# choyingw/SynergyNet

Hardware: AMD Instinct MI355X
Metric: faces/sec (120x120, 68-lmk + 53215-vert) (higher is better)
Workload: dtype f32 (fp16x2 split operands, fp32 accumulate)

## Files before the change

### synergynet_amd/csrc/fused_block_rm.hip

```cpp
#include "syn_internal.h"

#include <cstdlib>

namespace syn {

typedef float f32x4 __attribute__((ext_vector_type(4)));
typedef float f32x16 __attribute__((ext_vector_type(16)));
typedef unsigned u32x4 __attribute__((ext_vector_type(4)));
typedef _Float16 f16x8 __attribute__((ext_vector_type(8)));
typedef _Float16 f16x2 __attribute__((ext_vector_type(2)));

namespace {
constexpr int cdivr(int a, int b) { return (a + b - 1) / b; }

__device__ __forceinline__ void split2r(float x0, float x1, unsigned &a, unsigned &b) {
    a = __builtin_bit_cast(unsigned, __builtin_amdgcn_cvt_pkrtz(x0, x1));
    float r0, r1;
    asm("v_fma_mix_f32 %0, %1, -1.0, %2 op_sel_hi:[1,0,0]" : "=v"(r0) : "v"(a), "v"(x0));
    asm("v_fma_mix_f32 %0, %1, -1.0, %2 op_sel:[1,0,0] op_sel_hi:[1,0,0]" : "=v"(r1) : "v"(a), "v"(x1));
    b = __builtin_bit_cast(unsigned, __builtin_amdgcn_cvt_pkrtz(r0, r1));
}
__device__ __forceinline__ f32x16 mfma32r(u32x4 a, u32x4 b, f32x16 c) {
    return __builtin_amdgcn_mfma_f32_32x32x16_f16(__builtin_bit_cast(f16x8, a), __builtin_bit_cast(f16x8, b), c, 0, 0, 0);
}
__device__ __forceinline__ f32x16 mac3r(const u32x4 (&a)[2], const u32x4 (&b)[2], f32x16 c) {
// ... 14 lines not shown
struct RmCfg {
    static constexpr bool SVC2 = SVC2_;
    static constexpr int NSVW = SVC2_ ? 2 * U_ : U_;
    static constexpr int CIN = CIN_, HID = HID_, COUT = COUT_, H = H_, S = S_, NF = NF_, WPE = WPE_, U = U_;
    static constexpr bool RES = RES_;
    static constexpr bool LEAN = LEAN_;
    static constexpr int WREG = WREG_;
    static constexpr int KS = cdivr(CIN, 16);
    static constexpr int NG = cdivr(HID, 32);
    static constexpr int HIDP = NG * 32;
    static constexpr int NQ = COUT / 8;
    static constexpr int NB = S == 1 ? 1 : 2;
    static constexpr int HO = S == 2 ? H / 2 : H;
    static constexpr int NBD = NBD_, HB = HO / NBD;
    static constexpr int BSTEPS = S == 1 ? cdivr(HB + 2, 3) * 3 : 2 * (HB + 1);
    static_assert(HO % NBD == 0 && (NBD == 1 || !LEAN_), "bands: equal heights; not implemented for the one-slot (LEAN) sums");
    static_assert(!SVC2_ || NBD_ == 1, "two service waves per unit: implemented for the whole-face march");
    static constexpr int NW = NG, NCW = U * NG, NT = (NCW + NSVW) * 64;
    static constexpr int FR = NB * KS;
    static constexpr int XP_DW = FR * 2 * 256, PART_DW = NW * NQ * 256;
    static constexpr int PSLOTS = LEAN ? 1 : 2;
    static constexpr int UNIT_DW = 2 * XP_DW + PSLOTS * PART_DW;
    static constexpr int APL_DW = LEAN ? NG * 2 * 2 * 256 : 0;
    static constexpr int LDS_DW = U * UNIT_DW + 11 * HIDP + 32 + APL_DW;
    static_assert(COUT % 8 == 0 && COUT <= 32, "project tile");
    static_assert(S == 1 || H % 2 == 0, "stride-2 blocks have even input sizes");
    static_assert(S == 1 ? (NF == 1 ? H + 2 <= 32 : 2 * H + 2 <= 32) : (NF == 1 ? H / 2 + 1 <= 32 : H / 2 + 1 <= 16), "one image row per 32-lane block");
    static_assert(!RES || (S == 1 && CIN == COUT), "residual only on stride-1 same-width blocks");
    static_assert(!LEAN || S == 1, "LEAN is implemented for the stride-1 march");
    static_assert(WREG == 0 || (S == 1 && WREG <= 4), "the register-held filter is implemented for the stride-1 march");
    static_assert(S == 2 || H % 3 == 0, "row ring unrolled by 3");
    static_assert(NT <= 1024 && LDS_DW * 4 <= 160 * 1024, "workgroup size / LDS budget");
};

#define SYNR_LAP(i) do { if (PROF) { tn = __builtin_amdgcn_s_memtime(); pt_[i] += tn - tk; tk = tn; } } while (0)
#define SYNR_BARRIER() do { if (PROF) { const unsigned long long tb_ = __builtin_amdgcn_s_memtime(); busy_ += tb_ - tw_; __syncthreads(); tw_ = __builtin_amdgcn_s_memtime(); } else __syncthreads(); } while (0)

template <class C, bool PROF>
__device__ __forceinline__ void rm_block(unsigned *smem, const float *__restrict__ X, const unsigned *__restrict__ Ae3 ,
                           const unsigned *__restrict__ Ap3 , const float *__restrict__ e_shift,
                           const float *__restrict__ Wd , const float *__restrict__ d_shift,
                           const float *__restrict__ p_shift, float *__restrict__ Y, int B, int ub_begin, int ub_end, int ub_step ,
                           const float *__restrict__ scl_e , const float *__restrict__ scl_p,
                           unsigned long long *prof) {
    unsigned long long pt_[7] = {0, 0, 0, 0, 0, 0, 0}, tk = PROF ? __builtin_amdgcn_s_memtime() : 0ull, tn = 0, nsteps = 0;
    const unsigned long long t_begin = tk;
    unsigned long long busy_ = 0, tw_ = tk;
    constexpr int H = C::H, HO = C::HO, NW = C::NW, NT = C::NT;
    const int tid = threadIdx.x, lane = tid & 63;
    const int wave_wg = __builtin_amdgcn_readfirstlane(tid >> 6);
    const bool service = wave_wg >= C::NCW;
    const int uw = service ? (wave_wg - C::NCW) % C::U : wave_wg / NW;
    const bool svc_in = !C::SVC2 || wave_wg - C::NCW < C::U, svc_out = !C::SVC2 || wave_wg - C::NCW >= C::U;
    const int wave = service ? 0 : wave_wg % NW;
    unsigned *Xp = smem + uw * C::UNIT_DW;
    float *Part = reinterpret_cast<float *>(Xp + 2 * C::XP_DW);
    float *Filt = reinterpret_cast<float *>(smem + C::U * C::UNIT_DW);
    float *Esh = Filt + 10 * C::HIDP, *Psh = Esh + C::HIDP;
    unsigned *ApL = reinterpret_cast<unsigned *>(Psh + 32);
    constexpr int DSH = 9 * C::HIDP;
    const int j = lane & 31, h = lane >> 5;
    const int cb = wave * 32 + 4 * h;
    const int nq_live = (C::HID % 32 == 16 && wave == NW - 1) ? 2 : 4;

    int ia, icol[C::NB], oa, ocol;
    if (C::S == 1 && C::NF == 2) {
        ia = j > C::H; icol[0] = (j == 0 || j == C::H + 1) ? -1 : j - 1 - (C::H + 1) * ia; oa = ia; ocol = icol[0];
    } else if (C::S == 1) { ia = 0; icol[0] = j - 1; oa = 0; ocol = j - 1; }
    else if (C::NF == 1) { ia = 0; icol[0] = 2 * j - 1; icol[C::NB - 1] = 2 * j; oa = 0; ocol = j; }
    else { ia = j >> 4; icol[0] = 2 * (j & 15) - 1; icol[C::NB - 1] = 2 * (j & 15); oa = j >> 4; ocol = j & 15; }
    u32x4 ae[C::KS][2], ap[2][2];
    unsigned early_sink = 0;
    if (!service) {
#pragma unroll
        for (int s = 0; s < C::KS; ++s)
#pragma unroll
            for (int p = 0; p < 2; ++p) ae[s][p] = *(const u32x4 *)(Ae3 + ((size_t)(wave * C::KS + s) * 2 + p) * 256 + lane * 4);
        if (!C::LEAN)
#pragma unroll
            for (int s = 0; s < 2; ++s)
#pragma unroll
                for (int p = 0; p < 2; ++p) ap[s][p] = *(const u32x4 *)(Ap3 + ((size_t)(wave * 2 + s) * 2 + p) * 256 + lane * 4);
    } else if (svc_in && ub_begin < ub_end) {
        const int unit = ub_begin + uw, fu = C::NBD > 1 ? unit / C::NBD : unit, r0 = C::NBD > 1 ? (unit - fu * C::NBD) * C::HB : 0;
        const int f_in = fu * C::NF + ia, y0 = C::NBD > 1 ? (C::S == 1 ? r0 - 1 : 2 * (r0 - 1)) : 0;
#pragma unroll
        for (int b = 0; b < C::NB; ++b)
#pragma unroll
            for (int yy = 0; yy < 2; ++yy) {
                const int y = y0 + yy;
                if ((unsigned)icol[b] < (unsigned)H && f_in < B && (unsigned)y < (unsigned)H) {
                    const float *src = X + ((size_t)(f_in * H + y) * H + icol[b]) * C::CIN + 8 * h;
                    asm volatile("global_load_dword %0, %1, off" : "+v"(early_sink) : "v"(src) : "memory");
                }
            }
    }
    const float Se = scl_e[0], c6e = scl_e[1] * (1.0f / 6.0f), inv_sp = scl_p[1] * 6.0f;
    for (int i = tid; i < 9 * C::HIDP; i += NT) { const int c = i % C::HIDP; Filt[i] = c < C::HID ? Wd[(i / C::HIDP) * C::HID + c] : 0.f; }
    for (int i = tid; i < C::HIDP; i += NT) { Filt[DSH + i] = i < C::HID ? d_shift[i] * (1.0f / 6.0f) : 0.f; Esh[i] = i < C::HID ? e_shift[i] * Se : 0.f; }
    if (tid < 32) Psh[tid] = tid < C::COUT ? p_shift[tid] : 0.f;
    if (C::LEAN)
        for (int i = tid; i < C::APL_DW / 4; i += NT) *(u32x4 *)&ApL[4 * i] = *(const u32x4 *)&Ap3[4 * i];

    __syncthreads();
    l2_touch_done(early_sink);

    if (service) {
        __builtin_amdgcn_s_setprio(3);
        for (int ub = ub_begin; ub < ub_end; ub += ub_step) {
            const int unit = ub + uw;
            const int fu = C::NBD > 1 ? unit / C::NBD : unit, r0 = C::NBD > 1 ? (unit - fu * C::NBD) * C::HB : 0;
            const int f_in = fu * C::NF + ia, f_out = fu * C::NF + oa;
            const bool out_ok = (unsigned)ocol < (unsigned)HO && f_out < B;
            f32x4 xr[C::FR][2];
            auto load_row = [&](int y) {
#pragma unroll
                for (int fr = 0; fr < C::FR; ++fr) {
                    const int b = fr / C::KS, sk = fr % C::KS, c0 = 16 * sk + 8 * h;
                    xr[fr][0] = (f32x4){0.f, 0.f, 0.f, 0.f}; xr[fr][1] = xr[fr][0];
                    if (c0 + 8 <= C::CIN && (unsigned)icol[b] < (unsigned)H && f_in < B && (C::NBD == 1 || (unsigned)y < (unsigned)H)) {
                        const float *src = X + ((size_t)(f_in * H + y) * H + icol[b]) * C::CIN + c0;
                        xr[fr][0] = *(const f32x4 *)src; xr[fr][1] = *(const f32x4 *)(src + 4);
                    }
                }
            };
            auto store_row = [&](int slot) {
#pragma unroll
                for (int fr = 0; fr < C::FR; ++fr) {
                    u32x4 pc[2];
#pragma unroll
                    for (int t = 0; t < 2; ++t) {
                        unsigned a0, b0, a1, b1;
                        split2r(xr[fr][t][0], xr[fr][t][1], a0, b0);
                        split2r(xr[fr][t][2], xr[fr][t][3], a1, b1);
                        pc[0][2 * t] = a0; pc[0][2 * t + 1] = a1; pc[1][2 * t] = b0; pc[1][2 * t + 1] = b1;
                    }
                    unsigned *dst = Xp + (size_t)slot * C::XP_DW + fr * 512 + lane * 4;
#pragma unroll
                    for (int p = 0; p < 2; ++p) *(u32x4 *)(dst + p * 256) = pc[p];
                }
            };
            f32x4 res[C::RES ? C::NQ : 1];
            auto load_res = [&](int yo) {
                if (C::RES) {
#pragma unroll
                    for (int q = 0; q < C::NQ; ++q) {
                        res[q] = (f32x4){0.f, 0.f, 0.f, 0.f};
                        if (out_ok && yo >= 0 && yo < HO) res[q] = *(const f32x4 *)(X + ((size_t)(f_out * H + yo) * H + ocol) * C::CIN + 8 * q + 4 * h);
// ... 14 lines not shown
            };
            if (C::NBD > 1) {
                constexpr int NS = C::BSTEPS, HB = C::HB;
                const int gy0 = C::S == 1 ? r0 - 1 : 2 * (r0 - 1);
                load_row(gy0);
                store_row(0);
                load_row(gy0 + 1);
                SYNR_BARRIER();
                for (int k = 0; k < NS; ++k) {
                    if (C::S == 1) {
                        if (k >= 3 && k < HB + 3) reduce_row(r0 + k - 3, (k - 1) & 1);
                        if (k >= 2) load_res(r0 + k - 2);
                    } else {
                        if (!(k & 1) && k >= 4) reduce_row(r0 + (k >> 1) - 2, ((k >> 1) - 1) & 1);
                    }
                    if (k + 1 < NS) store_row((k + 1) & 1);
                    if (k + 2 < NS) load_row(gy0 + k + 2);
                    SYNR_BARRIER();
                }
                if (C::S == 2) reduce_row(r0 + HB - 1, HB & 1);
                else if (NS == HB + 2) reduce_row(r0 + HB - 1, (NS - 1) & 1);
                continue;
            }
            if (svc_in) { load_row(0); store_row(0); load_row(1); }
            SYNR_BARRIER();
            if (C::S == 1) {
                if (svc_out) load_res(0);
                constexpr int PM = C::PSLOTS - 1;
                for (int y = 0; y < H; ++y) {
                    if (svc_out && y >= 2) reduce_row(y - 2, y & PM);
                    if (C::LEAN) SYNR_BARRIER();
                    if (svc_out) load_res(y - 1);
                    if (svc_in && y + 1 < H) store_row((y + 1) & 1);
                    if (svc_in && y + 2 < H) load_row(y + 2);
                    SYNR_BARRIER();
                }
                if (svc_out) reduce_row(H - 2, (H - 2) & PM);
                if (C::LEAN) SYNR_BARRIER();
                if (svc_out) load_res(H - 1);
                SYNR_BARRIER();
                if (svc_out) reduce_row(H - 1, (H - 1) & PM);
            } else {
                for (int y = 0; y < H; ++y) {
                    if (svc_out && !(y & 1) && y >= 2) reduce_row((y >> 1) - 1, ((y >> 1) - 1) & 1);
                    if (svc_in && y + 1 < H) store_row((y + 1) & 1);
                    if (svc_in && y + 2 < H) load_row(y + 2);
                    SYNR_BARRIER();
                }
                if (svc_out) reduce_row(HO - 1, (HO - 1) & 1);
            }
        }
        if (PROF && lane == 0) atomicAdd(&prof[8 + wave_wg], busy_);
        return;
    }

    f32x4 wreg[C::WREG > 0 ? C::WREG : 1][9], wbase[C::WREG > 0 ? C::WREG : 1];
#pragma unroll
    for (int q = 0; q < C::WREG; ++q) {
#pragma unroll
        for (int k = 0; k < 9; ++k) wreg[q][k] = *(const f32x4 *)(Filt + cb + 8 * q + k * C::HIDP);
        wbase[q] = *(const f32x4 *)(Filt + cb + 8 * q + DSH);
    }
    for (int ub = ub_begin; ub < ub_end; ub += ub_step) {
        const int unit = ub + uw;
        const int fu = C::NBD > 1 ? unit / C::NBD : unit, r0 = C::NBD > 1 ? (unit - fu * C::NBD) * C::HB : 0;
        const int f_in = fu * C::NF + ia;
        float ehi[C::NB];
        float ehs[C::NB];
#pragma unroll
        for (int b = 0; b < C::NB; ++b) ehs[b] = ehi[b] = ((unsigned)icol[b] < (unsigned)H && f_in < B) ? c6e : 0.0f;
        auto row_ceiling = [&](int gy) {
#pragma unroll
            for (int b = 0; b < C::NB; ++b) ehs[b] = (unsigned)gy < (unsigned)H ? ehi[b] : 0.0f;
        };

        auto expand = [&](int slot, int b, f32x16 &e, int cbo) {
#pragma unroll
            for (int q = 0; q < 4; ++q) {
                const f32x4 sh = *(const f32x4 *)&Esh[cbo + 8 * q];
#pragma unroll
                for (int t = 0; t < 4; ++t) e[4 * q + t] = sh[t];
            }
#pragma unroll
            for (int s = 0; s < C::KS; ++s) {
                u32x4 xb[2];
                const unsigned *src = Xp + (size_t)slot * C::XP_DW + (b * C::KS + s) * 512 + lane * 4;
#pragma unroll
                for (int p = 0; p < 2; ++p) xb[p] = *(const u32x4 *)(src + p * 256);
                e = mac3r(ae[s], xb, e);
// ... 55 lines not shown
            for (int t = 0; t < 4; ++t) asm volatile("" : "+v"(d[4 * q + t]));
        };
        auto taps2 = [&](f32x16 &d, int q, const float *wq, int ta, int tb, const f32x4 &c4, const f32x4 &r4, bool init) {
            const f32x4 wa = *(const f32x4 *)(wq + ta * C::HIDP), wb = *(const f32x4 *)(wq + tb * C::HIDP);
            f32x4 base;
            if (init) base = *(const f32x4 *)(wq + DSH);
#pragma unroll
            for (int t = 0; t < 4; ++t) d[4 * q + t] = __builtin_fmaf(r4[t], wb[t], __builtin_fmaf(c4[t], wa[t], init ? base[t] : d[4 * q + t]));
#pragma unroll
            for (int t = 0; t < 4; ++t) asm volatile("" : "+v"(d[4 * q + t]));
        };
        auto taps1 = [&](f32x16 &d, int q, const float *wq, int ta, const f32x16 &e, bool last = false) {
            const f32x4 wa = *(const f32x4 *)(wq + ta * C::HIDP);
#pragma unroll
            for (int t = 0; t < 4; ++t) {
                const float v = __builtin_fmaf(e[4 * q + t], wa[t], d[4 * q + t]);
                d[4 * q + t] = last ? __builtin_amdgcn_fmed3f(v, 0.0f, 1.0f) : v;
            }
#pragma unroll
            for (int t = 0; t < 4; ++t) asm volatile("" : "+v"(d[4 * q + t]));
        };
        auto opaque_cb = [&]() { int c = cb; asm volatile("" : "+v"(c)); return c; };

        SYNR_BARRIER();

        if (C::S == 1) {
            f32x16 d0, d1, d2;
            {
                const int cbo = opaque_cb();
#pragma unroll
                for (int q = 0; q < 4; ++q) {
                    const f32x4 sh = *(const f32x4 *)(Filt + cbo + 8 * q + DSH);
#pragma unroll
                    for (int t = 0; t < 4; ++t) { d0[4 * q + t] = sh[t]; d1[4 * q + t] = 0.f; d2[4 * q + t] = 0.f; }
                }
            }
            auto step = [&](int xslot, bool fin, int pslot, f32x16 &dm, f32x16 &dc, f32x16 &dn) {
                SYNR_LAP(5);
                const int cbo = opaque_cb();
                f32x16 e;
                expand(xslot, 0, e, cbo);
                SYNR_LAP(1);
#pragma unroll
                for (int q = 0; q < 4; ++q) {
                    if (q >= nq_live) break;
                    f32x4 c4, l4, r4;
#pragma unroll
// ... 13 lines not shown
                SYNR_LAP(3);
                if (C::LEAN) SYNR_BARRIER();
                if (fin) finalize(dm, pslot);
                SYNR_LAP(4);
                SYNR_BARRIER();
                nsteps += 1;
            };
            if (C::NBD > 1) {
                auto bstep = [&](int k, f32x16 &dm, f32x16 &dc, f32x16 &dn) {
                    row_ceiling(r0 - 1 + k);
                    step(k & 1, k >= 2 && k < C::HB + 2, k & 1, dm, dc, dn);
                };
                for (int k = 0; k < C::BSTEPS; k += 3) {
                    bstep(k, d2, d0, d1);
                    bstep(k + 1, d0, d1, d2);
                    bstep(k + 2, d1, d2, d0);
                }
            } else {
                for (int y = 0; y < H; y += 3) {
                    step(y & 1, y >= 1, (y - 1) & (C::PSLOTS - 1), d2, d0, d1);
                    step((y + 1) & 1, true, y & (C::PSLOTS - 1), d0, d1, d2);
                    step((y + 2) & 1, true, (y + 1) & (C::PSLOTS - 1), d1, d2, d0);
                }
                if (C::LEAN) SYNR_BARRIER();
                finalize(d2, (H - 1) & (C::PSLOTS - 1), true);
                SYNR_BARRIER();
            }
        } else {
            f32x16 dcur, dnext;
            {
                const int cbo = opaque_cb();
#pragma unroll
                for (int q = 0; q < 4; ++q) {
                    const f32x4 sh = *(const f32x4 *)(Filt + cbo + 8 * q + DSH);
#pragma unroll
                    for (int t = 0; t < 4; ++t) { dcur[4 * q + t] = sh[t]; dnext[4 * q + t] = 0.f; }
                }
            }
            const int np = C::NBD > 1 ? C::HB + 1 : HO, p0 = C::NBD > 1 ? r0 - 1 : 0;
            for (int lp = 0; lp < np; ++lp) {
                const int yo = p0 + lp;
                {
                    if (C::NBD > 1) row_ceiling(2 * yo);
                    SYNR_LAP(5);
                    const int cbo = opaque_cb();
                    f32x16 e;
                    expand(0, 0, e, cbo);
#pragma unroll
// ... 29 lines not shown
#pragma unroll
                        for (int t = 0; t < 4; ++t) { c4[t] = e[4 * q + t]; r4[t] = from_right(c4[t]); }
                        taps2(dcur, q, Filt + cbo + 8 * q, 6, 8, c4, r4, false);
                        taps2(dnext, q, Filt + cbo + 8 * q, 0, 2, c4, r4, true);
                        __builtin_amdgcn_sched_barrier(0);
                    }
                    expand(1, 1, e, cbo);
#pragma unroll
                    for (int q = 0; q < 4; ++q) {
                        if (q >= nq_live) break;
                        taps1(dcur, q, Filt + cbo + 8 * q, 7, e, true);
                        taps1(dnext, q, Filt + cbo + 8 * q, 1, e);
                        __builtin_amdgcn_sched_barrier(0);
                    }
                    SYNR_LAP(3);
                    if (C::NBD == 1 || lp >= 1) finalize(dcur, lp & 1);
                    SYNR_LAP(4);
                    dcur = dnext;
                    SYNR_BARRIER();
                    nsteps += 1;
                }
            }
        }
    }
    if (PROF && lane == 0) atomicAdd(&prof[8 + wave_wg], busy_);
    if (PROF && tid == 0) {
        pt_[6] = __builtin_amdgcn_s_memtime() - t_begin;
        for (int i = 0; i < 7; ++i) atomicAdd(&prof[i], pt_[i]);
        atomicAdd(&prof[7], nsteps);
    }
}

template <class C, bool PROF = false>
__global__ __launch_bounds__(C::NT) __attribute__((amdgpu_waves_per_eu(C::WPE, C::WPE)))
void fused_block_rm_kernel(const float *__restrict__ X, const unsigned *__restrict__ Ae3, const unsigned *__restrict__ Ap3, const float *__restrict__ e_shift,
                           const float *__restrict__ Wd, const float *__restrict__ d_shift, const float *__restrict__ p_shift, float *__restrict__ Y, int B,
                           int n_units, const float *__restrict__ scl_e, const float *__restrict__ scl_p, unsigned long long *prof = nullptr) {
    __shared__ __attribute__((aligned(16))) unsigned smem[C::LDS_DW];
    rm_block<C, PROF>(smem, X, Ae3, Ap3, e_shift, Wd, d_shift, p_shift, Y, B, blockIdx.x * C::U, n_units, gridDim.x * C::U, scl_e, scl_p, prof);
}

struct RmStageArgs {
    const float *X; const unsigned *Ae3, *Ap3; const float *e_shift, *Wd, *d_shift, *p_shift; float *Y; const float *scl_e, *scl_p;
};
template <class CA, class CB>
__global__ __launch_bounds__(CA::NT) __attribute__((amdgpu_waves_per_eu(CA::WPE, CA::WPE)))
void fused_pair_rm_kernel(RmStageArgs a, RmStageArgs b, int B) {
    static_assert(CA::NT == CB::NT && CA::WPE == CB::WPE && CA::NBD == 1 && CB::NBD == 1, "one workgroup shape for both blocks; whole-face marches");
    constexpr int FA = CA::U * CA::NF, FB = CB::U * CB::NF, FG = FA > FB ? FA : FB;
    static_assert(FG % FA == 0 && FG % FB == 0, "a group is whole rounds of both blocks");
    __shared__ __attribute__((aligned(16))) unsigned smem[CA::LDS_DW > CB::LDS_DW ? CA::LDS_DW : CB::LDS_DW];
    const int nua = (B + CA::NF - 1) / CA::NF, nub = (B + CB::NF - 1) / CB::NF;
    {
        const int gq = blockIdx.x;
        const int ua = gq * (FG / CA::NF), ub = gq * (FG / CB::NF);
        rm_block<CA, false>(smem, a.X, a.Ae3, a.Ap3, a.e_shift, a.Wd, a.d_shift, a.p_shift, a.Y, B, ua, ua + FG / CA::NF < nua ? ua + FG / CA::NF : nua, CA::U,
                            a.scl_e, a.scl_p, nullptr);
        __builtin_amdgcn_fence(__ATOMIC_RELEASE, "workgroup");
        __syncthreads();
        __builtin_amdgcn_fence(__ATOMIC_ACQUIRE, "workgroup");
        rm_block<CB, false>(smem, b.X, b.Ae3, b.Ap3, b.e_shift, b.Wd, b.d_shift, b.p_shift, b.Y, B, ub, ub + FG / CB::NF < nub ? ub + FG / CB::NF : nub, CB::U,
                            b.scl_e, b.scl_p, nullptr);
    }
}

template <class C>
static void launch_rm(const FusedBlockArgs &a, int B, hipStream_t s, int wgs_per_cu) {
    const int n_units = (B + C::NF - 1) / C::NF * C::NBD;
    const int cap = 256 * wgs_per_cu, wgs = (n_units + C::U - 1) / C::U;
    const int grid = wgs < cap ? wgs : cap;
    if (a.prof)
        fused_block_rm_kernel<C, true><<<grid, C::NT, 0, s>>>(a.X, a.Arm_e, a.Arm_p, a.e_shift, a.Wd, a.d_shift, a.p_shift, a.Y, B, n_units, a.scl_e, a.scl_p, a.prof);
    else
        fused_block_rm_kernel<C><<<grid, C::NT, 0, s>>>(a.X, a.Arm_e, a.Arm_p, a.e_shift, a.Wd, a.d_shift, a.p_shift, a.Y, B, n_units, a.scl_e, a.scl_p);
}

template <int U> using R2 = RmCfg< 16,  96,  24, 60, 2, 1, false, (U == 4 ? 4 : 3), U>;
template <int U> using R3 = RmCfg< 24, 144,  24, 30, 1, 1, true,  3, U, false, 1>;
template <int U> using R4 = RmCfg< 24, 144,  32, 30, 2, 2, false, 3, U>;
template <int U> using R5 = RmCfg< 32, 192,  32, 15, 1, 2, true,  4, U, true, 0, 1, true>;
template <int U, int NBD> using R2b = RmCfg< 16,  96,  24, 60, 2, 1, false, 3, U, false, 0, NBD>;
template <int U, int NBD> using R3b = RmCfg< 24, 144,  24, 30, 1, 1, true,  3, U, false, 1, NBD>;
constexpr int kBand2Min = 40, kBand3Min = 96;

template <class CA, class CB>
static void launch_pair(const FusedBlockArgs &a, const FusedBlockArgs &b, int B, hipStream_t s) {
    constexpr int FA = CA::U * CA::NF, FB = CB::U * CB::NF, FG = FA > FB ? FA : FB;
    const int n_groups = (B + FG - 1) / FG;
    fused_pair_rm_kernel<CA, CB><<<n_groups, CA::NT, 0, s>>>(RmStageArgs{a.X, a.Arm_e, a.Arm_p, a.e_shift, a.Wd, a.d_shift, a.p_shift, a.Y, a.scl_e, a.scl_p},
                                                        RmStageArgs{b.X, b.Arm_e, b.Arm_p, b.e_shift, b.Wd, b.d_shift, b.p_shift, b.Y, b.scl_e, b.scl_p}, B);
}
bool launch_fused_pair_rm(int first, const FusedBlockArgs &a, const FusedBlockArgs &b, int B, hipStream_t s) {
    static const bool on56 = test_knob("rm_pair56", 1) != 0, on34 = test_knob("rm_pair34", 1) != 0;
    if (B < 513 || a.prof || b.prof) return false;
    if (!a.Arm_e || !a.Arm_p || !a.scl_e || !a.scl_p || !b.Arm_e || !b.Arm_p || !b.scl_e || !b.scl_p) return false;
    if (first == 5 && on56) { launch_pair<R5<2>, R5<2>>(a, b, B, s); return true; }
    if (first == 3 && on34 && (B + 3) / 4 <= 256) { launch_pair<R3<2>, R4<2>>(a, b, B, s); return true; }
    return false;
}

bool launch_fused_block_rm(int feature, const FusedBlockArgs &a, int B, hipStream_t s) {
    if (!a.Arm_e || !a.Arm_p || !a.scl_e || !a.scl_p) return false;
    static const bool bands2 = test_knob("rm_band2", 1) != 0, bands3 = test_knob("rm_band3", 1) != 0;
    switch (feature) {
        case 2:
            if (B >= 513) { launch_rm<R2<4>>(a, B, s, 1); return true; }
            if (B >= 352) { launch_rm<R2<2>>(a, B, s, 1); return true; }
            if (bands2 && B >= kBand2Min) { launch_rm<R2b<1, 6>>(a, B, s, 3); return true; }
            return false;
        case 3:
            if (B >= 448) { launch_rm<R3<2>>(a, B, s, 1); return true; }
            if (B >= 200) { launch_rm<R3<1>>(a, B, s, 1); return true; }
            if (bands3 && B >= kBand3Min) { launch_rm<R3b<2, 3>>(a, B, s, 1); return true; }
            return false;
        case 4:
            if (B >= 513) { launch_rm<R4<2>>(a, B, s, 1); return true; }
            if (B >= 480) { launch_rm<R4<1>>(a, B, s, 1); return true; }
            return false;
        case 5:
        case 6:
// ... 8 lines not shown
```

### synergynet_amd/csrc/syn_internal.h

```cpp
#pragma once
#include <hip/hip_runtime.h>
#include <stddef.h>
#include <stdint.h>

namespace syn {

#ifdef __HIPCC__
__device__ __forceinline__ void l2_touch(const void *base, unsigned bytes, unsigned gi, unsigned nth, unsigned &sink) {
    for (unsigned ofs = gi * 128u; ofs < bytes; ofs += nth * 128u) {
        const char *p = static_cast<const char *>(base) + ofs;
        asm volatile("global_load_dword %0, %1, off" : "+v"(sink) : "v"(p) : "memory");
    }
}
__device__ __forceinline__ void l2_touch_done(unsigned &sink) { asm volatile("s_waitcnt vmcnt(0)" : "+v"(sink) :: "memory"); }
#endif

long long test_knob(const char *name, long long dflt);
bool test_knob_set(const char *name);

constexpr int kImg = 120;
constexpr int kParam = 62;
constexpr int kPool = 1280;
constexpr int kBasisK = 52;
constexpr int kVertTile = 32;
// ... 17 lines not shown
    const float *X;
    const float *We, *e_scale, *e_shift;
    const float *Wd, *d_scale, *d_shift;
    const float *Wp, *p_scale, *p_shift;
    float *Y;
    unsigned long long *prof = nullptr;
    const unsigned *We3 = nullptr, *Wp3 = nullptr;
    const float *scl_e = nullptr, *scl_p = nullptr;
    const unsigned *Arm_e = nullptr, *Arm_p = nullptr;
    const unsigned *Alb_p = nullptr;
    const unsigned *Alb_e = nullptr;
    const float *Tlb = nullptr;
    const unsigned *Glb = nullptr;
    float *scratch = nullptr;
    size_t scratch_floats = 0;
};
bool launch_fused_block(int feature, const FusedBlockArgs &a, int B, hipStream_t s);
constexpr int early_block_hc(int hid) { return hid % 32 == 0 ? 32 : 48; }
bool launch_fused_block_early(int feature, const FusedBlockArgs &a, int B, hipStream_t s);
constexpr int rm_expand_dwords(int cin, int hid) { return ((hid + 31) / 32) * ((cin + 15) / 16) * 512; }
constexpr int rm_project_dwords(int hid) { return ((hid + 31) / 32) * 2 * 512; }
bool launch_fused_block_rm(int feature, const FusedBlockArgs &a, int B, hipStream_t s);
bool launch_fused_pair_rm(int first, const FusedBlockArgs &a, const FusedBlockArgs &b, int B, hipStream_t s);
bool launch_fused_pair_f16(const FusedBlockArgs &a5, const FusedBlockArgs &a6, int B, hipStream_t s);
constexpr int lb_project_dwords(int hid, int cout) { return (hid / 32) * (cout / 16) * 512; }
constexpr int lb_expand_dwords(int cin, int hid) { return (hid / 16) * (cin / 32) * 512; }
constexpr int lb_table_floats(int hid) { return (hid / 32) * 12 * 32; }
bool launch_fused_block_lb(int feature, const FusedBlockArgs &a, int B, hipStream_t s);
int lb_chain_mode(int B, bool small = true);
bool launch_fused_chain_lb(const FusedBlockArgs *a, int first, int n_blocks, int B, hipStream_t s);
constexpr int lb4_group_dwords(int cin, int cout) { return (2 * (cin / 32) * 512 + (cout / 16) * 512 + 512 + 2047) / 2048 * 2048; }
bool launch_fused_block_lb4(int feature, const FusedBlockArgs &a, int B, hipStream_t s);
bool launch_fused_chain_lb4(const FusedBlockArgs *a, int B, hipStream_t s);
bool launch_fused_block_f16(int feature, const FusedBlockArgs &a, int B, hipStream_t s);

void launch_stem_block1(const float *img_nchw, const uint8_t *img_hwc_u8, const float *w0, const unsigned *w0b3, const float *s0,
                        const float *b0, const float *wd, const float *sd, const float *bd, const float *wp_pk,
                        const float *sp, const float *bp, float *Y, int B, hipStream_t s);

constexpr int rm_stem_set_dwords() { return 3 * 2 * 256 + 32 + 4; }
constexpr int rm_stem_dwords() { return 2 * rm_stem_set_dwords(); }
bool launch_stem_rm(const uint8_t *img8, const unsigned *As3, const float *s_shift, const float *Wd, const float *d_shift,
                    const unsigned *Ap3, const float *p_shift, const float *scl_p, float *Y, int B, hipStream_t s);
bool launch_stem_rm_f32(const float *img, const unsigned *As3, const float *s_shift, const float *Wd, const float *d_shift,
                        const unsigned *Ap3, const float *p_shift, const float *scl_p, float *Y, int B, hipStream_t s);

// ... 161 lines not shown
```

### synergynet_amd/csrc/synergy_abi.hip

```cpp
#include "../../include/synergy_hip.h"

#include <algorithm>
#include <cmath>
#include <cstdarg>
#include <cstdio>
#include <cstdlib>
#include <cstring>
#include <dlfcn.h>
#include <string>
#include <vector>

#include "syn_internal.h"
#include "bcast_protocol.h"

namespace {

thread_local std::string g_err;

int fail(int code, const char *fmt, ...) {
    char buf[512];
    va_list ap;
    va_start(ap, fmt);
    vsnprintf(buf, sizeof buf, fmt, ap);
    va_end(ap);
// ... 616 lines not shown
                syn::FusedBlockArgs a{xin, P + E.dst_wpk, P + E.dst_scale, P + E.dst_shift, P + D.dst_wpk, P + D.dst_scale, P + D.dst_shift,
                                      P + Pj.dst_wpk, P + Pj.dst_scale, P + Pj.dst_shift, yout};
                if (prof_feature == E.feature) a.prof = prof;
                const bool ok1 = !((u1 >> E.feature) & 1u), ok16 = !((u16 >> E.feature) & 1u);
                if (h->fusion >= 2 && ok1 && E.dst_wb3 && Pj.dst_wb3) {
                    a.We3 = reinterpret_cast<const unsigned *>(P + E.dst_wb3);
                    a.Wp3 = reinterpret_cast<const unsigned *>(P + Pj.dst_wb3);
                }
                if (h->fusion >= 2 && E.dst_scl && Pj.dst_scl) { a.scl_e = P + E.dst_scl; a.scl_p = P + Pj.dst_scl; }
                if (h->fusion >= 2 && ok1 && E.dst_wrm && Pj.dst_wrm && ((h->early_rm >> (E.feature <= 4 ? E.feature - 2 : E.feature)) & 1)) {
                    a.Arm_e = reinterpret_cast<const unsigned *>(P + E.dst_wrm);
                    a.Arm_p = reinterpret_cast<const unsigned *>(P + Pj.dst_wrm);
                }
                if (h->fusion >= 2 && ok16 && a.We3 && Pj.dst_wlb && E.dst_tlb && (h->early_rm & 128)) {
                    a.Alb_p = reinterpret_cast<const unsigned *>(P + Pj.dst_wlb);
                    a.Alb_e = reinterpret_cast<const unsigned *>(P + E.dst_weh);
                    a.Tlb = P + E.dst_tlb;
                }
                if (h->fusion >= 2 && ok16 && E.dst_glb && (h->early_rm & 256)) a.Glb = reinterpret_cast<const unsigned *>(P + E.dst_glb);
                a.scratch = H2; a.scratch_floats = (size_t)B * n.max_hidden;
                return a;
            };
            syn::FusedBlockArgs a = block_args(li, X, Y);
            if ((L.feature == 3 || L.feature == 5) && (a.Arm_e || (L.feature == 5 && a.We3)) && prof_feature < 0 && (stop_feature < 0 || stop_feature >= L.feature + 1) && li + 6 <= nl &&
                n.layers[li + 3].kind == PW && n.layers[li + 3].relu6 && n.layers[li + 3].feature == L.feature + 1) {
                const Layer &Pb = n.layers[li + 5];
                const size_t in_a = (size_t)L.cin * L.hin * L.hin, out_b = (size_t)Pb.cout * Pb.hout * Pb.hout;
                float *const out2 = (L.feature == 3 && in_a + out_b <= n.max_io) ? X + (size_t)B * in_a : (L.feature == 5 ? X : nullptr);
                const syn::FusedBlockArgs b = block_args(li + 3, Y, out2);
                if (out2 && ((a.Arm_e && b.Arm_e && syn::launch_fused_pair_rm(L.feature, a, b, B, s)) ||
                             (L.feature == 5 && a.We3 && b.We3 && B < 513 && syn::launch_fused_pair_f16(a, b, B, s)))) {
                    X = out2;
                    li += 5;
                    mark(100 * L.feature + L.feature + 1);
                    if (stop_feature == L.feature + 1) {
                        const Layer &Lp = n.layers[li];
                        HIP_TRY(hipMemcpyAsync(feature_out, X, (size_t)B * Lp.cout * Lp.hout * Lp.hout * sizeof(float), hipMemcpyDeviceToDevice, s));
                        return SYN_OK;
                    }
                    continue;
                }
            }
            if (L.feature == 17 && a.Glb && stop_feature < 0 && prof_feature < 0 && !((u1 >> 18) & 1u) && syn::launch_lb4_sliced17_deferred(a, B, s, &head_sliced)) {
                have_head_sliced = true;
                float *t = X; X = Y; Y = t;
                li += 2;
                mark(L.feature);
// ... 2641 lines not shown
```

Before: 994,600.

## Hand over between fused pair blocks without a barrier, prestaging next block's inputs

For the fused pair kernel whose two blocks share one configuration (R5 pair), the first block now stages the second block's constants into a separate LDS region up front. During its last round it also loads the next block's expand/project weights into registers and its first input rows. The second block then starts without reloading weights or constants and without the full workgroup barrier, using workgroup fences at chosen rows instead. This hides the start-up latency of the second stage at the cost of more LDS and more intricate ordering. Optional timestamp profiling is added behind a knob.

```diff
diff --git a/synergynet_amd/csrc/fused_block_rm.hip b/synergynet_amd/csrc/fused_block_rm.hip
--- a/synergynet_amd/csrc/fused_block_rm.hip
+++ b/synergynet_amd/csrc/fused_block_rm.hip
@@ -1,6 +1,7 @@
 #include "syn_internal.h"
 
 #include <cstdlib>
+#include <type_traits>
 
 namespace syn {
 
@@ -61,7 +62,8 @@
     static constexpr int PSLOTS = LEAN ? 1 : 2;
     static constexpr int UNIT_DW = 2 * XP_DW + PSLOTS * PART_DW;
     static constexpr int APL_DW = LEAN ? NG * 2 * 2 * 256 : 0;
-    static constexpr int LDS_DW = U * UNIT_DW + 11 * HIDP + 32 + APL_DW;
+    static constexpr int CONST_DW = 11 * HIDP + 32 + APL_DW;
+    static constexpr int LDS_DW = U * UNIT_DW + CONST_DW;
     static_assert(COUT % 8 == 0 && COUT <= 32, "project tile");
     static_assert(S == 1 || H % 2 == 0, "stride-2 blocks have even input sizes");
     static_assert(S == 1 ? (NF == 1 ? H + 2 <= 32 : 2 * H + 2 <= 32) : (NF == 1 ? H / 2 + 1 <= 32 : H / 2 + 1 <= 16), "one image row per 32-lane block");
@@ -75,17 +77,60 @@
 #define SYNR_LAP(i) do { if (PROF) { tn = __builtin_amdgcn_s_memtime(); pt_[i] += tn - tk; tk = tn; } } while (0)
 #define SYNR_BARRIER() do { if (PROF) { const unsigned long long tb_ = __builtin_amdgcn_s_memtime(); busy_ += tb_ - tw_; __syncthreads(); tw_ = __builtin_amdgcn_s_memtime(); } else __syncthreads(); } while (0)
 
-template <class C, bool PROF>
-__device__ __forceinline__ void rm_block(unsigned *smem, const float *__restrict__ X, const unsigned *__restrict__ Ae3 ,
+struct RmStageArgs {
+    const float *X; const unsigned *Ae3, *Ap3; const float *e_shift, *Wd, *d_shift, *p_shift; float *Y; const float *scl_e, *scl_p;
+};
+template <class C> struct RmCarry {
+    u32x4 ae[C::KS][2], ap[2][2];
+};
+struct RmHoProf { unsigned long long t_fin = 0, pair = 0, round = 0; };
+enum : int {
+    RM_PRE = 1,
+    RM_NEXT = 2,
+    RM_STAMP = 4
+};
+template <class C>
+__device__ __forceinline__ void rm_stage_consts(unsigned *cst, const unsigned *__restrict__ Ap3, const float *__restrict__ e_shift, const float *__restrict__ Wd,
+                                                const float *__restrict__ d_shift, const float *__restrict__ p_shift, float Se, int tid) {
+    float *Filt = reinterpret_cast<float *>(cst), *Esh = Filt + 10 * C::HIDP, *Psh = Esh + C::HIDP;
+    unsigned *ApL = reinterpret_cast<unsigned *>(Psh + 32);
+    constexpr int DSH = 9 * C::HIDP, NT = C::NT;
+    for (int i = tid; i < 9 * C::HIDP; i += NT) { const int c = i % C::HIDP; Filt[i] = c < C::HID ? Wd[(i / C::HIDP) * C::HID + c] : 0.f; }
+    for (int i = tid; i < C::HIDP; i += NT) { Filt[DSH + i] = i < C::HID ? d_shift[i] * (1.0f / 6.0f) : 0.f; Esh[i] = i < C::HID ? e_shift[i] * Se : 0.f; }
+    if (tid < 32) Psh[tid] = tid < C::COUT ? p_shift[tid] : 0.f;
+    if (C::LEAN)
+        for (int i = tid; i < C::APL_DW / 4; i += NT) *(u32x4 *)&ApL[4 * i] = *(const u32x4 *)&Ap3[4 * i];
+}
+template <class C>
+__device__ __forceinline__ void rm_load_ae(u32x4 (&ae)[C::KS][2], const unsigned *__restrict__ Ae3, int wave, int lane) {
+#pragma unroll
+    for (int s = 0; s < C::KS; ++s)
+#pragma unroll
+        for (int p = 0; p < 2; ++p) ae[s][p] = *(const u32x4 *)(Ae3 + ((size_t)(wave * C::KS + s) * 2 + p) * 256 + lane * 4);
+}
+template <class C>
+__device__ __forceinline__ void rm_load_ap(u32x4 (&ap)[2][2], const unsigned *__restrict__ Ap3, int wave, int lane) {
+    if (!C::LEAN)
+#pragma unroll
+        for (int s = 0; s < 2; ++s)
+#pragma unroll
+            for (int p = 0; p < 2; ++p) ap[s][p] = *(const u32x4 *)(Ap3 + ((size_t)(wave * 2 + s) * 2 + p) * 256 + lane * 4);
+}
+
+template <class C, bool PROF, int MODE = 0>
+__device__ __forceinline__ void rm_block(unsigned *smem, unsigned *cst, const float *__restrict__ X, const unsigned *__restrict__ Ae3 ,
                            const unsigned *__restrict__ Ap3 , const float *__restrict__ e_shift,
                            const float *__restrict__ Wd , const float *__restrict__ d_shift,
                            const float *__restrict__ p_shift, float *__restrict__ Y, int B, int ub_begin, int ub_end, int ub_step ,
                            const float *__restrict__ scl_e , const float *__restrict__ scl_p,
-                           unsigned long long *prof) {
+                           unsigned long long *prof, RmCarry<C> &cur, unsigned *cstN, const RmStageArgs &nx, RmHoProf &hp) {
+    static_assert(!(MODE & (RM_NEXT | RM_PRE)) || (C::S == 1 && C::NBD == 1 && C::CIN == C::COUT && C::H >= 11),
+                  "hand-over between two blocks of one configuration: the stride-1 whole-face march, output rows = input rows (H: see the fences)");
+    constexpr bool HAND_NEXT = (MODE & RM_NEXT) != 0, CARRIED = (MODE & RM_PRE) != 0;
     unsigned long long pt_[7] = {0, 0, 0, 0, 0, 0, 0}, tk = PROF ? __builtin_amdgcn_s_memtime() : 0ull, tn = 0, nsteps = 0;
     const unsigned long long t_begin = tk;
     unsigned long long busy_ = 0, tw_ = tk;
-    constexpr int H = C::H, HO = C::HO, NW = C::NW, NT = C::NT;
+    constexpr int H = C::H, HO = C::HO, NW = C::NW;
     const int tid = threadIdx.x, lane = tid & 63;
     const int wave_wg = __builtin_amdgcn_readfirstlane(tid >> 6);
     const bool service = wave_wg >= C::NCW;
@@ -94,7 +139,7 @@
     const int wave = service ? 0 : wave_wg % NW;
     unsigned *Xp = smem + uw * C::UNIT_DW;
     float *Part = reinterpret_cast<float *>(Xp + 2 * C::XP_DW);
-    float *Filt = reinterpret_cast<float *>(smem + C::U * C::UNIT_DW);
+    float *Filt = reinterpret_cast<float *>(cst);
     float *Esh = Filt + 10 * C::HIDP, *Psh = Esh + C::HIDP;
     unsigned *ApL = reinterpret_cast<unsigned *>(Psh + 32);
     constexpr int DSH = 9 * C::HIDP;
@@ -108,18 +153,12 @@
     } else if (C::S == 1) { ia = 0; icol[0] = j - 1; oa = 0; ocol = j - 1; }
     else if (C::NF == 1) { ia = 0; icol[0] = 2 * j - 1; icol[C::NB - 1] = 2 * j; oa = 0; ocol = j; }
     else { ia = j >> 4; icol[0] = 2 * (j & 15) - 1; icol[C::NB - 1] = 2 * (j & 15); oa = j >> 4; ocol = j & 15; }
-    u32x4 ae[C::KS][2], ap[2][2];
+    u32x4 (&ae)[C::KS][2] = cur.ae, (&ap)[2][2] = cur.ap;
     unsigned early_sink = 0;
-    if (!service) {
-#pragma unroll
-        for (int s = 0; s < C::KS; ++s)
-#pragma unroll
-            for (int p = 0; p < 2; ++p) ae[s][p] = *(const u32x4 *)(Ae3 + ((size_t)(wave * C::KS + s) * 2 + p) * 256 + lane * 4);
-        if (!C::LEAN)
-#pragma unroll
-            for (int s = 0; s < 2; ++s)
-#pragma unroll
-                for (int p = 0; p < 2; ++p) ap[s][p] = *(const u32x4 *)(Ap3 + ((size_t)(wave * 2 + s) * 2 + p) * 256 + lane * 4);
+    if (MODE & RM_PRE) {
+    } else if (!service) {
+        rm_load_ae<C>(ae, Ae3, wave, lane);
+        rm_load_ap<C>(ap, Ap3, wave, lane);
     } else if (svc_in && ub_begin < ub_end) {
         const int unit = ub_begin + uw, fu = C::NBD > 1 ? unit / C::NBD : unit, r0 = C::NBD > 1 ? (unit - fu * C::NBD) * C::HB : 0;
         const int f_in = fu * C::NF + ia, y0 = C::NBD > 1 ? (C::S == 1 ? r0 - 1 : 2 * (r0 - 1)) : 0;
@@ -135,34 +174,37 @@
             }
     }
     const float Se = scl_e[0], c6e = scl_e[1] * (1.0f / 6.0f), inv_sp = scl_p[1] * 6.0f;
-    for (int i = tid; i < 9 * C::HIDP; i += NT) { const int c = i % C::HIDP; Filt[i] = c < C::HID ? Wd[(i / C::HIDP) * C::HID + c] : 0.f; }
-    for (int i = tid; i < C::HIDP; i += NT) { Filt[DSH + i] = i < C::HID ? d_shift[i] * (1.0f / 6.0f) : 0.f; Esh[i] = i < C::HID ? e_shift[i] * Se : 0.f; }
-    if (tid < 32) Psh[tid] = tid < C::COUT ? p_shift[tid] : 0.f;
-    if (C::LEAN)
-        for (int i = tid; i < C::APL_DW / 4; i += NT) *(u32x4 *)&ApL[4 * i] = *(const u32x4 *)&Ap3[4 * i];
-
-    __syncthreads();
-    l2_touch_done(early_sink);
+    if (!(MODE & RM_PRE)) {
+        rm_stage_consts<C>(cst, Ap3, e_shift, Wd, d_shift, p_shift, Se, tid);
+        if (MODE & RM_NEXT) rm_stage_consts<C>(cstN, nx.Ap3, nx.e_shift, nx.Wd, nx.d_shift, nx.p_shift, nx.scl_e[0], tid);
+
+        __syncthreads();
+        l2_touch_done(early_sink);
+    }
+    bool first_round = true;
 
     if (service) {
         __builtin_amdgcn_s_setprio(3);
+        bool staged = CARRIED;
         for (int ub = ub_begin; ub < ub_end; ub += ub_step) {
             const int unit = ub + uw;
             const int fu = C::NBD > 1 ? unit / C::NBD : unit, r0 = C::NBD > 1 ? (unit - fu * C::NBD) * C::HB : 0;
             const int f_in = fu * C::NF + ia, f_out = fu * C::NF + oa;
             const bool out_ok = (unsigned)ocol < (unsigned)HO && f_out < B;
+            const bool hand = HAND_NEXT && ub + ub_step >= ub_end;
             f32x4 xr[C::FR][2];
-            auto load_row = [&](int y) {
+            auto load_row_of = [&](const float *Xs, int f, int y) {
 #pragma unroll
                 for (int fr = 0; fr < C::FR; ++fr) {
                     const int b = fr / C::KS, sk = fr % C::KS, c0 = 16 * sk + 8 * h;
                     xr[fr][0] = (f32x4){0.f, 0.f, 0.f, 0.f}; xr[fr][1] = xr[fr][0];
-                    if (c0 + 8 <= C::CIN && (unsigned)icol[b] < (unsigned)H && f_in < B && (C::NBD == 1 || (unsigned)y < (unsigned)H)) {
-                        const float *src = X + ((size_t)(f_in * H + y) * H + icol[b]) * C::CIN + c0;
+                    if (c0 + 8 <= C::CIN && (unsigned)icol[b] < (unsigned)H && f < B && (C::NBD == 1 || (unsigned)y < (unsigned)H)) {
+                        const float *src = Xs + ((size_t)(f * H + y) * H + icol[b]) * C::CIN + c0;
                         xr[fr][0] = *(const f32x4 *)src; xr[fr][1] = *(const f32x4 *)(src + 4);
                     }
                 }
             };
+            auto load_row = [&](int y) { load_row_of(X, f_in, y); };
             auto store_row = [&](int slot) {
 #pragma unroll
                 for (int fr = 0; fr < C::FR; ++fr) {
@@ -223,19 +265,29 @@
                 else if (NS == HB + 2) reduce_row(r0 + HB - 1, (NS - 1) & 1);
                 continue;
             }
-            if (svc_in) { load_row(0); store_row(0); load_row(1); }
-            SYNR_BARRIER();
+            if (!staged) {
+                if (svc_in) { load_row(0); store_row(0); load_row(1); }
+                SYNR_BARRIER();
+            }
             if (C::S == 1) {
                 if (svc_out) load_res(0);
                 constexpr int PM = C::PSLOTS - 1;
+                constexpr int FS = H & 1;
                 for (int y = 0; y < H; ++y) {
+                    if (hand && svc_out && y == H - 3) __builtin_amdgcn_fence(__ATOMIC_RELEASE, "workgroup");
+                    if (hand && svc_in && y == H - 2) __builtin_amdgcn_fence(__ATOMIC_ACQUIRE, "workgroup");
+                    if (CARRIED && svc_out && y == 2) __builtin_amdgcn_fence(__ATOMIC_RELEASE, "workgroup");
+                    if (CARRIED && svc_in && y == 3) __builtin_amdgcn_fence(__ATOMIC_ACQUIRE, "workgroup");
                     if (svc_out && y >= 2) reduce_row(y - 2, y & PM);
                     if (C::LEAN) SYNR_BARRIER();
                     if (svc_out) load_res(y - 1);
-                    if (svc_in && y + 1 < H) store_row((y + 1) & 1);
+                    if (svc_in && y + 1 < H && !(staged && y == 0)) store_row((y + 1) & 1);
                     if (svc_in && y + 2 < H) load_row(y + 2);
+                    if (hand && svc_in && y == H - 2) load_row_of(nx.X, f_in, FS);
+                    if (hand && svc_in && y == H - 1) { store_row(FS); load_row_of(nx.X, f_in, 1 - FS); }
                     SYNR_BARRIER();
                 }
+                if (hand && svc_in) store_row(1 - FS);
                 if (svc_out) reduce_row(H - 2, (H - 2) & PM);
                 if (C::LEAN) SYNR_BARRIER();
                 if (svc_out) load_res(H - 1);
@@ -250,6 +302,7 @@
                 }
                 if (svc_out) reduce_row(HO - 1, (HO - 1) & 1);
             }
+            staged = hand;
         }
         if (PROF && lane == 0) atomicAdd(&prof[8 + wave_wg], busy_);
         return;
@@ -262,10 +315,12 @@
         for (int k = 0; k < 9; ++k) wreg[q][k] = *(const f32x4 *)(Filt + cb + 8 * q + k * C::HIDP);
         wbase[q] = *(const f32x4 *)(Filt + cb + 8 * q + DSH);
     }
+    bool staged = CARRIED;
     for (int ub = ub_begin; ub < ub_end; ub += ub_step) {
         const int unit = ub + uw;
         const int fu = C::NBD > 1 ? unit / C::NBD : unit, r0 = C::NBD > 1 ? (unit - fu * C::NBD) * C::HB : 0;
         const int f_in = fu * C::NF + ia;
+        const bool hand = HAND_NEXT && ub + ub_step >= ub_end;
         float ehi[C::NB];
         float ehs[C::NB];
 #pragma unroll
@@ -367,7 +422,11 @@
         };
         auto opaque_cb = [&]() { int c = cb; asm volatile("" : "+v"(c)); return c; };
 
-        SYNR_BARRIER();
+        if (!staged) SYNR_BARRIER();
+        if ((MODE & RM_STAMP) && wave_wg == 0) {
+            if (hp.t_fin) (first_round ? hp.pair : hp.round) += __builtin_amdgcn_s_memtime() - hp.t_fin;
+            first_round = false;
+        }
 
         if (C::S == 1) {
             f32x16 d0, d1, d2;
@@ -427,8 +486,11 @@
                     step((y + 1) & 1, true, y & (C::PSLOTS - 1), d0, d1, d2);
                     step((y + 2) & 1, true, (y + 1) & (C::PSLOTS - 1), d1, d2, d0);
                 }
+                if (hand) rm_load_ae<C>(ae, nx.Ae3, wave, lane);
                 if (C::LEAN) SYNR_BARRIER();
                 finalize(d2, (H - 1) & (C::PSLOTS - 1), true);
+                if (hand) rm_load_ap<C>(ap, nx.Ap3, wave, lane);
+                if ((MODE & RM_STAMP) && wave_wg == 0) hp.t_fin = __builtin_amdgcn_s_memtime();
                 SYNR_BARRIER();
             }
         } else {
@@ -504,6 +566,7 @@
                 }
             }
         }
+        staged = hand;
     }
     if (PROF && lane == 0) atomicAdd(&prof[8 + wave_wg], busy_);
     if (PROF && tid == 0) {
@@ -519,30 +582,56 @@
                            const float *__restrict__ Wd, const float *__restrict__ d_shift, const float *__restrict__ p_shift, float *__restrict__ Y, int B,
                            int n_units, const float *__restrict__ scl_e, const float *__restrict__ scl_p, unsigned long long *prof = nullptr) {
     __shared__ __attribute__((aligned(16))) unsigned smem[C::LDS_DW];
-    rm_block<C, PROF>(smem, X, Ae3, Ap3, e_shift, Wd, d_shift, p_shift, Y, B, blockIdx.x * C::U, n_units, gridDim.x * C::U, scl_e, scl_p, prof);
-}
-
-struct RmStageArgs {
-    const float *X; const unsigned *Ae3, *Ap3; const float *e_shift, *Wd, *d_shift, *p_shift; float *Y; const float *scl_e, *scl_p;
-};
-template <class CA, class CB>
+    RmCarry<C> cur;
+    RmHoProf hp;
+    const RmStageArgs none{};
+    rm_block<C, PROF>(smem, smem + C::U * C::UNIT_DW, X, Ae3, Ap3, e_shift, Wd, d_shift, p_shift, Y, B, blockIdx.x * C::U, n_units, gridDim.x * C::U, scl_e, scl_p, prof,
+                      cur, nullptr, none, hp);
+}
+
+template <class CA, class CB, bool HO, bool STAMP = false>
 __global__ __launch_bounds__(CA::NT) __attribute__((amdgpu_waves_per_eu(CA::WPE, CA::WPE)))
-void fused_pair_rm_kernel(RmStageArgs a, RmStageArgs b, int B) {
+void fused_pair_rm_kernel(RmStageArgs a, RmStageArgs b, int B, unsigned long long *prof) {
     static_assert(CA::NT == CB::NT && CA::WPE == CB::WPE && CA::NBD == 1 && CB::NBD == 1, "one workgroup shape for both blocks; whole-face marches");
+    static_assert(!HO || std::is_same<CA, CB>::value, "the hand-over form: two blocks of one configuration");
     constexpr int FA = CA::U * CA::NF, FB = CB::U * CB::NF, FG = FA > FB ? FA : FB;
     static_assert(FG % FA == 0 && FG % FB == 0, "a group is whole rounds of both blocks");
-    __shared__ __attribute__((aligned(16))) unsigned smem[CA::LDS_DW > CB::LDS_DW ? CA::LDS_DW : CB::LDS_DW];
+    constexpr int UA = CA::U * CA::UNIT_DW, UB = CB::U * CB::UNIT_DW;
+    constexpr int LDS_DW = HO ? UA + CA::CONST_DW + CB::CONST_DW : (CA::LDS_DW > CB::LDS_DW ? CA::LDS_DW : CB::LDS_DW);
+    static_assert(LDS_DW * 4 <= 160 * 1024, "LDS budget");
+    __shared__ __attribute__((aligned(16))) unsigned smem[LDS_DW];
+    constexpr int ST = STAMP ? RM_STAMP : 0;
+    const unsigned long long t_begin = STAMP ? __builtin_amdgcn_s_memtime() : 0ull;
+    RmHoProf hp;
     const int nua = (B + CA::NF - 1) / CA::NF, nub = (B + CB::NF - 1) / CB::NF;
     {
         const int gq = blockIdx.x;
         const int ua = gq * (FG / CA::NF), ub = gq * (FG / CB::NF);
-        rm_block<CA, false>(smem, a.X, a.Ae3, a.Ap3, a.e_shift, a.Wd, a.d_shift, a.p_shift, a.Y, B, ua, ua + FG / CA::NF < nua ? ua + FG / CA::NF : nua, CA::U,
-                            a.scl_e, a.scl_p, nullptr);
-        __builtin_amdgcn_fence(__ATOMIC_RELEASE, "workgroup");
-        __syncthreads();
-        __builtin_amdgcn_fence(__ATOMIC_ACQUIRE, "workgroup");
-        rm_block<CB, false>(smem, b.X, b.Ae3, b.Ap3, b.e_shift, b.Wd, b.d_shift, b.p_shift, b.Y, B, ub, ub + FG / CB::NF < nub ? ub + FG / CB::NF : nub, CB::U,
-                            b.scl_e, b.scl_p, nullptr);
+        const int ua_end = ua + FG / CA::NF < nua ? ua + FG / CA::NF : nua, ub_end = ub + FG / CB::NF < nub ? ub + FG / CB::NF : nub;
+        if constexpr (!HO) {
+            RmCarry<CA> ca;
+            RmCarry<CB> cb;
+            rm_block<CA, false, ST>(smem, smem + UA, a.X, a.Ae3, a.Ap3, a.e_shift, a.Wd, a.d_shift, a.p_shift, a.Y, B, ua, ua_end, CA::U, a.scl_e, a.scl_p, nullptr,
+                                    ca, nullptr, b, hp);
+            __builtin_amdgcn_fence(__ATOMIC_RELEASE, "workgroup");
+            __syncthreads();
+            __builtin_amdgcn_fence(__ATOMIC_ACQUIRE, "workgroup");
+            rm_block<CB, false, ST>(smem, smem + UB, b.X, b.Ae3, b.Ap3, b.e_shift, b.Wd, b.d_shift, b.p_shift, b.Y, B, ub, ub_end, CB::U, b.scl_e, b.scl_p, nullptr,
+                                    cb, nullptr, b, hp);
+        } else {
+            RmCarry<CA> c;
+            unsigned *const cstA = smem + UA, *const cstB = cstA + CA::CONST_DW;
+            rm_block<CA, false, ST | RM_NEXT>(smem, cstA, a.X, a.Ae3, a.Ap3, a.e_shift, a.Wd, a.d_shift, a.p_shift, a.Y, B, ua, ua_end, CA::U, a.scl_e, a.scl_p, nullptr,
+                                              c, cstB, b, hp);
+            rm_block<CB, false, ST | RM_PRE>(smem, cstB, b.X, b.Ae3, b.Ap3, b.e_shift, b.Wd, b.d_shift, b.p_shift, b.Y, B, ub, ub_end, CB::U, b.scl_e, b.scl_p, nullptr,
+                                             c, nullptr, b, hp);
+        }
+    }
+    if (STAMP && threadIdx.x == 0) {
+        atomicAdd(&prof[0], hp.pair);
+        atomicAdd(&prof[1], hp.round);
+        atomicAdd(&prof[6], __builtin_amdgcn_s_memtime() - t_begin);
+        atomicAdd(&prof[7], 1ull);
     }
 }
 
@@ -566,18 +655,32 @@
 constexpr int kBand2Min = 40, kBand3Min = 96;
 
 template <class CA, class CB>
-static void launch_pair(const FusedBlockArgs &a, const FusedBlockArgs &b, int B, hipStream_t s) {
+static void launch_pair(const FusedBlockArgs &a, const FusedBlockArgs &b, int B, hipStream_t s, bool handover) {
     constexpr int FA = CA::U * CA::NF, FB = CB::U * CB::NF, FG = FA > FB ? FA : FB;
     const int n_groups = (B + FG - 1) / FG;
-    fused_pair_rm_kernel<CA, CB><<<n_groups, CA::NT, 0, s>>>(RmStageArgs{a.X, a.Arm_e, a.Arm_p, a.e_shift, a.Wd, a.d_shift, a.p_shift, a.Y, a.scl_e, a.scl_p},
-                                                        RmStageArgs{b.X, b.Arm_e, b.Arm_p, b.e_shift, b.Wd, b.d_shift, b.p_shift, b.Y, b.scl_e, b.scl_p}, B);
+    const RmStageArgs ra{a.X, a.Arm_e, a.Arm_p, a.e_shift, a.Wd, a.d_shift, a.p_shift, a.Y, a.scl_e, a.scl_p},
+                      rb{b.X, b.Arm_e, b.Arm_p, b.e_shift, b.Wd, b.d_shift, b.p_shift, b.Y, b.scl_e, b.scl_p};
+    if constexpr (std::is_same<CA, CB>::value) {
+        if (handover) {
+            if (a.prof) fused_pair_rm_kernel<CA, CB, true, true><<<n_groups, CA::NT, 0, s>>>(ra, rb, B, a.prof);
+            else fused_pair_rm_kernel<CA, CB, true><<<n_groups, CA::NT, 0, s>>>(ra, rb, B, nullptr);
+            return;
+        }
+    }
+    if (a.prof) fused_pair_rm_kernel<CA, CB, false, true><<<n_groups, CA::NT, 0, s>>>(ra, rb, B, a.prof);
+    else fused_pair_rm_kernel<CA, CB, false><<<n_groups, CA::NT, 0, s>>>(ra, rb, B, nullptr);
+}
+bool rm_pair_profiled() {
+    static const bool on = test_knob("rm_pair_prof", 0) != 0;
+    return on;
 }
 bool launch_fused_pair_rm(int first, const FusedBlockArgs &a, const FusedBlockArgs &b, int B, hipStream_t s) {
     static const bool on56 = test_knob("rm_pair56", 1) != 0, on34 = test_knob("rm_pair34", 1) != 0;
-    if (B < 513 || a.prof || b.prof) return false;
+    static const bool handover = test_knob("rm_pair_handover", 1) != 0;
+    if (B < 513 || b.prof || (a.prof && !rm_pair_profiled())) return false;
     if (!a.Arm_e || !a.Arm_p || !a.scl_e || !a.scl_p || !b.Arm_e || !b.Arm_p || !b.scl_e || !b.scl_p) return false;
-    if (first == 5 && on56) { launch_pair<R5<2>, R5<2>>(a, b, B, s); return true; }
-    if (first == 3 && on34 && (B + 3) / 4 <= 256) { launch_pair<R3<2>, R4<2>>(a, b, B, s); return true; }
+    if (first == 5 && on56) { launch_pair<R5<2>, R5<2>>(a, b, B, s, handover); return true; }
+    if (first == 3 && on34 && (B + 3) / 4 <= 256) { launch_pair<R3<2>, R4<2>>(a, b, B, s, handover); return true; }
     return false;
 }
 
diff --git a/synergynet_amd/csrc/syn_internal.h b/synergynet_amd/csrc/syn_internal.h
--- a/synergynet_amd/csrc/syn_internal.h
+++ b/synergynet_amd/csrc/syn_internal.h
@@ -63,6 +63,7 @@
 constexpr int rm_project_dwords(int hid) { return ((hid + 31) / 32) * 2 * 512; }
 bool launch_fused_block_rm(int feature, const FusedBlockArgs &a, int B, hipStream_t s);
 bool launch_fused_pair_rm(int first, const FusedBlockArgs &a, const FusedBlockArgs &b, int B, hipStream_t s);
+bool rm_pair_profiled();
 bool launch_fused_pair_f16(const FusedBlockArgs &a5, const FusedBlockArgs &a6, int B, hipStream_t s);
 constexpr int lb_project_dwords(int hid, int cout) { return (hid / 32) * (cout / 16) * 512; }
 constexpr int lb_expand_dwords(int cin, int hid) { return (hid / 16) * (cin / 32) * 512; }
diff --git a/synergynet_amd/csrc/synergy_abi.hip b/synergynet_amd/csrc/synergy_abi.hip
--- a/synergynet_amd/csrc/synergy_abi.hip
+++ b/synergynet_amd/csrc/synergy_abi.hip
@@ -662,7 +662,7 @@
                 return a;
             };
             syn::FusedBlockArgs a = block_args(li, X, Y);
-            if ((L.feature == 3 || L.feature == 5) && (a.Arm_e || (L.feature == 5 && a.We3)) && prof_feature < 0 && (stop_feature < 0 || stop_feature >= L.feature + 1) && li + 6 <= nl &&
+            if ((L.feature == 3 || L.feature == 5) && (a.Arm_e || (L.feature == 5 && a.We3)) && (prof_feature < 0 || (prof_feature == L.feature && syn::rm_pair_profiled())) && (stop_feature < 0 || stop_feature >= L.feature + 1) && li + 6 <= nl &&
                 n.layers[li + 3].kind == PW && n.layers[li + 3].relu6 && n.layers[li + 3].feature == L.feature + 1) {
                 const Layer &Pb = n.layers[li + 5];
                 const size_t in_a = (size_t)L.cin * L.hin * L.hin, out_b = (size_t)Pb.cout * Pb.hout * Pb.hout;
```

Result: no change. 994,900, median of 3 (+0.0%).
